# 583phoenix-hue/Airfoil-CFD-Tool

Hardware: AMD Instinct MI355X
Metric: MLUPS on 4096² fp32 D2Q9 at 1/2/4/8 MI355X; achieved % HBM3E peak (higher is better)
Workload: dtype f32

## Files before the change

airfoil-cfd-tool_amd/csrc/step_march.hpp:

```cpp
#pragma once
#include <hip/hip_runtime.h>
#include <stdint.h>
#include <algorithm>
#include <vector>
#include "step_fast.hpp"

#ifndef WT_LOAD_AUX
#define WT_LOAD_AUX 2
#endif
#ifndef WT_STORE_AUX
#define WT_STORE_AUX 2
#endif

namespace wt {

static constexpr int MARCH_MAX_CHUNK = 60;
static constexpr int MARCH3_MAX_CHUNK = 124;
static inline int march_max_len(int depth) { return depth == 4 ? MARCH3_MAX_CHUNK - 3 : (depth == 3 ? MARCH3_MAX_CHUNK : MARCH_MAX_CHUNK); }

struct ClassMask { unsigned long long lo, hi; };
__device__ __forceinline__ bool cm_bit(const ClassMask &m, int idx) { return (((idx < 64) ? (m.lo >> idx) : (m.hi >> (idx - 64))) & 1ULL) != 0; }

enum : uint8_t { WC_FAST = 0, WC_GENERAL = 1, WC_SOLID = 2 };

// ... 241 lines not shown

template <typename T, int S>
__device__ __forceinline__ void march_load_aligned(const MarchAddr<T, S> &a, int col, MV<T, S> (&fin)[9])
{
    fin[0] = bload<T, S>(a.rs, a.voff, lat_off(a, 0, col, 0));
    fin[1] = bload<T, S>(a.rs, a.voff, lat_off(a, 1, col - 1, 0));
    fin[3] = bload<T, S>(a.rs, a.voff, lat_off(a, 3, col + 1, 0));
    fin[2] = bload<T, S>(a.rs, a.voff, lat_off(a, 2, col, 0));
    fin[5] = bload<T, S>(a.rs, a.voff, lat_off(a, 5, col - 1, 0));
    fin[6] = bload<T, S>(a.rs, a.voff, lat_off(a, 6, col + 1, 0));
    fin[4] = bload<T, S>(a.rs, a.voff, lat_off(a, 4, col, 0));
    fin[7] = bload<T, S>(a.rs, a.voff, lat_off(a, 7, col + 1, 0));
    fin[8] = bload<T, S>(a.rs, a.voff, lat_off(a, 8, col - 1, 0));
}

template <int S> __device__ __forceinline__ uint32_t load_site_bytes(const uint8_t *p)
{
    if constexpr (S == 4) return *reinterpret_cast<const uint32_t *>(p);
    else if constexpr (S == 2) return *reinterpret_cast<const uint16_t *>(p);
    else return *p;
}

struct SiteBytes { uint32_t v[2]; };
template <int S, bool OVL> __device__ __forceinline__ int site_row(int j0, int ny)
{
    if constexpr (OVL) return j0 < 0 ? 0 : (j0 > ny - S ? ny - S : j0);
    else return j0;
}
template <typename T, int S, bool OVL = false>
__device__ __forceinline__ SiteBytes site_bytes_load(const MarchParams<T> &p, int col, int j0)
{
    const int c = col < 0 ? 0 : (col > p.g.nxl - 1 ? p.g.nxl - 1 : col);
    const int jb = site_row<S, OVL>(j0, p.g.ny);
    SiteBytes r;
    r.v[0] = load_site_bytes<S>(p.mask + (long)(c + 1) * p.g.pitch + jb);
    r.v[1] = load_site_bytes<S>(p.bcode + (long)c * p.g.pitch + jb);
    return r;
}

static constexpr int MARCH_FD_PACKED = 4;
typedef float f2v __attribute__((ext_vector_type(2)));
__device__ __forceinline__ f2v div2_ieee(f2v a, f2v b)
{
    bool s0, s1, dummy;
    const f2v ds = {__builtin_amdgcn_div_scalef(a[0], b[0], false, &dummy), __builtin_amdgcn_div_scalef(a[1], b[1], false, &dummy)};
    const f2v ns = {__builtin_amdgcn_div_scalef(a[0], b[0], true, &s0), __builtin_amdgcn_div_scalef(a[1], b[1], true, &s1)};
    const f2v rc = {__builtin_amdgcn_rcpf(ds[0]), __builtin_amdgcn_rcpf(ds[1])};
    const f2v one = {1.0f, 1.0f};
    const f2v f0 = __builtin_elementwise_fma(-ds, rc, one);
    const f2v f1 = __builtin_elementwise_fma(f0, rc, rc);
    const f2v mu = ns * f1;
// ... 254 lines not shown
#pragma unroll
    for (int k = 0; k < 9; k++) {
        const unsigned soff = lat_off(a, k, col, 0) - (OVL ? 256u : 0u);
        __builtin_amdgcn_raw_ptr_buffer_load_lds(a.rs, (lds_void_p)(buf + 512 * k), 4, a.voff_dma, soff, 0, 0);
        __builtin_amdgcn_raw_ptr_buffer_load_lds(a.rs, (lds_void_p)(buf + 512 * k), 4, a.voff_dma, soff, 256, 0);
    }
}
template <typename T, int S>
__device__ __forceinline__ MV<T, S> own_read(const char *buf, int k, int lane)
{
    MV<T, S> o;
    const u2v x = *reinterpret_cast<const u2v *>(buf + 512 * k + 8 * lane);
    __builtin_memcpy(&o, &x, 8);
    return o;
}

template <bool BODY, int FD, typename T, int S, bool OWN_LDS = false>
__device__ __forceinline__ void march_step1(const MarchParams<T> &p, const MarchAddr<T, S> &a, int x, int j0, bool far_win, bool nonfast, bool allsolid,
                                            const T (&feq0)[9], MV<T, S> (&in)[9], MV<T, S> (&G)[9], const uint32_t *pre = nullptr, const char *own_buf = nullptr)
{
    MV<T, S> mac[3];
    if (BODY) {
        const Geom &g = p.g;
        const int gi = x + g.gi0;
#ifdef WT_EXP_NO_OWN
        auto own = [&](int k) { return in[k]; };
#else
        auto own = [&](int k) {
            if constexpr (OWN_LDS) return own_read<T, S>(own_buf, k, a.lane);
            else return bload<T, S>(a.rs, a.voff, lat_off(a, k, x, 0));
        };
#endif
        if (__builtin_expect(gi <= 0 || gi >= g.nx_g - 1 || nonfast, 0)) {
            uint32_t solid4 = 0, code4 = 0;
            if (nonfast) {
                if (pre) { solid4 = pre[0]; code4 = pre[1]; }
                else {
                    solid4 = load_site_bytes<S>(p.mask + (long)(x + 1) * g.pitch + site_row<S, (FD & MARCH_FD_OVL) != 0>(j0, g.ny));
                    code4 = load_site_bytes<S>(p.bcode + (long)x * g.pitch + site_row<S, (FD & MARCH_FD_OVL) != 0>(j0, g.ny));
                }
            }
            const bool any_solid = __ballot(solid4 != 0) != 0ULL;
            if (gi <= 0) {
#pragma unroll
                for (int k = 0; k < 9; k++) G[k] = mv_splat<T, S>(feq0[k]);
            } else if (gi >= g.nx_g - 1) {
#pragma unroll
                for (int k = 0; k < 9; k++) G[k] = bload<T, S>(a.rs, a.voff, lat_off(a, k, x - 1, 0));
            } else if (allsolid) {
#pragma unroll
                for (int k = 0; k < 9; k++) G[k] = own(opp_of(k));
                return;
            } else {
                march_bounce<T, S>(in, code4, own);
                march_collide_general<T, S, FD, false>(in, solid4, j0, g.ny, p.fdv, p.tau, p.U0, feq0, G, mac);
                return;
            }
            if (any_solid) march_solid<T, S, false>(G, mac, solid4, own);
            return;
        }
    }
    march_collide<T, S, FD, false>(in, p.fdv, p.tau, G, mac);
    if (far_win) march_far_rows<T, S, false>(j0, p.g.ny, p.U0, feq0, G, mac);
}

struct MarchRange { int i_begin, i_end, outlet_after; };
static inline MarchRange march_range(const Geom &g)
{
    MarchRange r;
    r.i_begin = (g.gi0 == 0) ? 0 : 1;
    r.i_end = g.nxl - 1;
    r.outlet_after = (g.gi0 + g.nxl == g.nx_g) ? 1 : 0;
    return r;
// ... 128 lines not shown
```

airfoil-cfd-tool_amd/csrc/step_march3.hpp:

```cpp
#pragma once
#include "step_march.hpp"

namespace wt {

static constexpr int M3_SREC = 80;
static constexpr int M3_SHALF = 40;
static constexpr int M3_HL = 32;
static constexpr int HL_COLS = 60;
static constexpr int H3_COLS = HL_COLS, H4_COLS = HL_COLS;


__global__ __launch_bounds__(256) void k_seam_flags3(const uint8_t *__restrict__ mask, const uint8_t *__restrict__ bcode, uint8_t *__restrict__ flags3,
                                                     Geom g, int nwin, int win)
{
    const long total = (long)(nwin - 1) * g.nxl;
    const long t = (long)blockIdx.x * 256 + threadIdx.x;
    if (t >= total) return;
    const int x = (int)(t % g.nxl);
    const int b = 1 + (int)(t / g.nxl);
    const uint8_t *m = mask + g.pitch;
    const int gi = x + g.gi0;
    unsigned f = 0;
    for (int r4 = 0; r4 < 4; r4++) {
        const int j = win * b - 2 + r4;
// ... 281 lines not shown
                                            const T (&feq0)[9], const MV<T, S> (&m158)[3], const MV<T, S> (&Gc)[9], const MV<T, S> (&Gn)[9], T hv,
                                            MV<T, S> (&out)[9], MV<T, S> (&mac)[3], const uint32_t *pre = nullptr)
{
    typedef MV<T, S> V3;
    const Geom &g = p.g;
    constexpr bool OVL = (FD & MARCH_FD_OVL) != 0;
    V3 fin[9];
    fin[0] = Gc[0]; fin[1] = m158[0]; fin[3] = Gn[3];
    fin[2] = m_below_x<LB, OVL>(Gc[2], hv); fin[5] = m_below_x<LB + 1, OVL>(m158[1], hv); fin[6] = m_below_x<LB + 2, OVL>(Gn[6], hv);
    fin[4] = m_above_x<LB, OVL>(Gc[4], hv); fin[8] = m_above_x<LB + 2, OVL>(m158[2], hv); fin[7] = m_above_x<LB + 1, OVL>(Gn[7], hv);
    if (BODY) {
        const int gi = c + g.gi0;
        if (__builtin_expect(gi <= 0 || nf, 0)) {
            auto ownc = [&](int k) { return Gc[k]; };
            uint32_t solid4 = 0, code4 = 0;
            if (nf) {
                if (pre) { solid4 = pre[0]; code4 = pre[1]; }
                else {
                    solid4 = load_site_bytes<S>(p.mask + (long)(c + 1) * g.pitch + site_row<S, OVL>(j0, g.ny));
                    code4 = load_site_bytes<S>(p.bcode + (long)c * g.pitch + site_row<S, OVL>(j0, g.ny));
                }
            }
            const bool any_solid = __ballot(solid4 != 0) != 0ULL;
            if (gi <= 0) {
#pragma unroll
                for (int k = 0; k < 9; k++) out[k] = mv_splat<T, S>(feq0[k]);
                if (WANT_MACRO) { mac[0] = mv_splat<T, S>(T(1)); mac[1] = mv_splat<T, S>(p.U0); mac[2] = mv_splat<T, S>(T(0)); }
            } else if (allsolid) {
#pragma unroll
                for (int k = 0; k < 9; k++) out[k] = Gc[k];
                if (WANT_MACRO) { mac[0] = mv_splat<T, S>(T(1)); mac[1] = mv_splat<T, S>(T(0)); mac[2] = mv_splat<T, S>(T(0)); }
            } else {
                march_bounce<T, S>(fin, code4, ownc);
                march_collide_general<T, S, FD, WANT_MACRO>(fin, solid4, j0, g.ny, p.fdv, p.tau, p.U0, feq0, out, mac);
            }
            if (any_solid && (gi <= 0 || allsolid)) march_solid<T, S, WANT_MACRO>(out, mac, solid4, ownc);
            return;
// ... 87 lines not shown

template <bool BODY, bool EMIT, int FD, typename T, int S>
__device__ __forceinline__ void march_unit3(const MarchParams<T> &p, March3Addr<T, S> &m, __amdgpu_buffer_rsrc_t rh, unsigned hoff,
                                            int ia, int ib, int uflags, int j0, int lane, bool far_win, ClassMask nonfast_m,
                                            ClassMask solid_m, const T (&feq0)[9])
{
    constexpr bool OVLF = (FD & MARCH_FD_OVL) != 0;
    typedef MV<T, S> V3;
    constexpr unsigned HREC = M3_HL * sizeof(T);
    const Geom &g = p.g;
    const MarchAddr<T, S> &a = m.a;
#define NONFAST(x) (BODY && cm_bit(nonfast_m, (x) - ia + 2))
#define ALLSOLID(x) (BODY && cm_bit(solid_m, (x) - ia + 2))
#define OWN_BUF(x) (a.own_lds + ((x) & 1) * OWN_LDS_BYTES)
#define OWN_NOW(x) do { if (BODY && NONFAST(x)) own_prefetch<T, S, OVLF>(a, (x), OWN_BUF(x)); } while (0)
#define STEP1(x, in, G) march_step1<BODY, FD, T, S, BODY>(p, a, (x), j0, far_win, NONFAST(x), ALLSOLID(x), feq0, in, G, nullptr, OWN_BUF(x))
#define STEP1P(x, in, G, sb) march_step1<BODY, FD, T, S, BODY>(p, a, (x), j0, far_win, NONFAST(x), ALLSOLID(x), feq0, in, G, BODY ? (sb).v : nullptr, OWN_BUF(x))
    const bool outlet = BODY && (uflags & MU_OUTLET_AFTER) != 0;
    const int xend = outlet ? ib : ib + 1;
    V3 s1m[3], s1c[9];
    V3 s2m[3], s2c[9];
    V3 in[9], G1[9], G2[9], mac[3];
#pragma unroll
    for (int k = 0; k < 9; k++) { s1c[k] = mv_splat<T, S>(feq0[k]); s2c[k] = s1c[k]; }
    s1m[0] = s1c[1]; s1m[1] = s1c[5]; s1m[2] = s1c[8];
    s2m[0] = s1c[1]; s2m[1] = s1c[5]; s2m[2] = s1c[8];
    T hv2 = halo_load_x<OVLF, T>(rh, hoff, (unsigned)(ia - 2 > 0 ? ia - 2 : 0) * HREC);
    T hv1 = halo_load_x<OVLF, T>(rh, hoff, (unsigned)(ia - 1 > 0 ? ia - 1 : 0) * HREC);
    T hv0 = halo_load_x<OVLF, T>(rh, hoff, (unsigned)ia * HREC);
    if (!BODY || ia - 2 + g.gi0 >= 0) {
        OWN_NOW(ia - 2);
        march_load_aligned(a, ia - 2, in);
        march_align_in<OVLF>(in, lane, hv2);
        STEP1(ia - 2, in, s1c);
    }
    s1m[0] = s1c[1]; s1m[1] = s1c[5]; s1m[2] = s1c[8];
    if (!BODY || ia - 1 + g.gi0 >= 0) {
        OWN_NOW(ia - 1);
        march_load_aligned(a, ia - 1, in);
        march_align_in<OVLF>(in, lane, hv1);
        STEP1(ia - 1, in, s1c);
    }
    OWN_NOW(ia);
    march_load_aligned(a, ia, in);
    SiteBytes sb0{{0, 0}}, sb1{{0, 0}}, sb2{{0, 0}};
    if (BODY) { sb0 = site_bytes_load<T, S, OVLF>(p, ia, j0); sb1 = site_bytes_load<T, S, OVLF>(p, ia - 1, j0); sb2 = site_bytes_load<T, S, OVLF>(p, ia - 2, j0); wait_for_bytes(sb0); wait_for_bytes(sb1); wait_for_bytes(sb2); }
    wait_for_column(in, hv0, hv1, hv2);
    int seam_col = -1;
#ifdef WT_M3_STAMPS
    unsigned long long st_[8] = {0, 0, 0, 0, 0, 0, 0, 0}, tprev_ = __builtin_amdgcn_s_memtime();
#endif
#pragma unroll 1
    for (int x = ia; x <= xend; x++) {
        V3 nxt[9];
        if (BODY && x + 1 <= xend && NONFAST(x + 1)) own_prefetch<T, S, OVLF>(a, x + 1, OWN_BUF(x + 1));
        march_load_aligned(a, (x + 1 <= xend) ? x + 1 : x, nxt);
        const bool has2 = x - 2 >= ia;
        const int c1 = x - 1, c2 = x - 2;
        const T hvn = halo_load_x<OVLF, T>(rh, hoff, (unsigned)(x + 1) * HREC);
        SiteBytes sbn{{0, 0}};
        if (BODY) sbn = site_bytes_load<T, S, OVLF>(p, x + 1, j0);
        const Seam3 sp = seam3_fetch<OVLF>(m);
        M3_STAMP(0);
        march_align_in<OVLF>(in, lane, hv0);
        STEP1P(x, in, G1, sb0);
        M3_STAMP(1);
        march_stage<BODY, false, FD, 0>(p, c1, j0, lane, far_win, NONFAST(c1), ALLSOLID(c1), feq0, s1m, s1c, G1, hv1, G2, mac, BODY ? sb1.v : nullptr);
#ifdef WT_M3_STAMPS
        pin_after(G2);
#endif
        M3_STAMP(2);
        V3 out[9];
        march_stage<BODY, EMIT, FD, 4>(p, c2, j0, lane, far_win, NONFAST(c2), ALLSOLID(c2), feq0, s2m, s2c, G2, hv2, out, mac, BODY ? sb2.v : nullptr);
        pin_after(out);
        M3_STAMP(3);
        wait_for_column(nxt, hvn);
        if (BODY) { wait_for_bytes(sbn); sb2 = sb1; sb1 = sb0; sb0 = sbn; }
#ifdef WT_M3_STAMPS
        asm volatile("s_waitcnt vmcnt(0)" ::: "memory");
#endif
        M3_STAMP(4);
        hv2 = hv1; hv1 = hv0; hv0 = hvn;
        march3_store<EMIT, OVLF>(m, has2 ? a.voff_st : p.lat_bytes, has2 ? c2 : 0, out, mac);
        seam3_flush<OVLF>(m, seam_col, sp);
        M3_STAMP(5);
        seam_col = has2 ? c2 : seam_col;
        if (BODY && outlet && x == xend) break;
        s2m[0] = s2c[1]; s2m[1] = s2c[5]; s2m[2] = s2c[8];
        s1m[0] = s1c[1]; s1m[1] = s1c[5]; s1m[2] = s1c[8];
#pragma unroll
        for (int k = 0; k < 9; k++) { s2c[k] = G2[k]; s1c[k] = G1[k]; in[k] = nxt[k]; }
    }
#ifdef WT_M3_STAMPS
    if (!BODY && lane == 0) {
        for (int i = 0; i < 6; i++) atomicAdd(&g_m3_stamps[i], st_[i]);
        atomicAdd(&g_m3_stamps[6], (unsigned long long)(xend - ia + 1));
        atomicAdd(&g_m3_stamps[7], 1ULL);
    }
#endif
    if (BODY && outlet) {
        const int co = ib;
        uint32_t solid4 = 0;
        if (NONFAST(co)) solid4 = load_site_bytes<S>(p.mask + (long)(co + 1) * g.pitch + site_row<S, OVLF>(j0, g.ny));
        const bool any_solid = __ballot(solid4 != 0) != 0ULL;
        V3 L2o[9], out[9];
#pragma unroll
        for (int k = 0; k < 9; k++) L2o[k] = s1c[k];
        if (any_solid) { auto own1 = [&](int k) { return G1[k]; }; march_solid<T, S, false>(L2o, mac, solid4, own1); }
        V3 t2m[3];
        t2m[0] = s2c[1]; t2m[1] = s2c[5]; t2m[2] = s2c[8];
        const T hv2t = halo_load_x<OVLF, T>(rh, hoff, (unsigned)(co - 1) * HREC);
        Seam3 sp = seam3_fetch<OVLF>(m);
        march_stage<BODY, EMIT, FD, 4>(p, co - 1, j0, lane, far_win, NONFAST(co - 1), ALLSOLID(co - 1), feq0, t2m, G2, L2o, hv2t, out, mac);
        march3_store<EMIT, OVLF>(m, a.voff_st, co - 1, out, mac);
        seam3_flush<OVLF>(m, seam_col, sp);
        seam_col = co - 1;
#pragma unroll
        for (int k = 0; k < 9; k++) out[k] = G2[k];
        if (EMIT) march_outlet_macro(G2, mac);
        if (any_solid) { auto own2 = [&](int k) { return L2o[k]; }; march_solid<T, S, EMIT>(out, mac, solid4, own2); }
        sp = seam3_fetch<OVLF>(m);
        march3_store<EMIT, OVLF>(m, a.voff_st, co, out, mac);
        seam3_flush<OVLF>(m, seam_col, sp);
        seam_col = co;
    }
    seam3_flush<OVLF>(m, seam_col, seam3_fetch<OVLF>(m));
#undef NONFAST
#undef ALLSOLID
#undef STEP1
#undef STEP1P
#undef OWN_BUF
#undef OWN_NOW
}

template <bool BODY, bool EMIT, int FD, typename T, int S>
__device__ __forceinline__ void march_unit4(const MarchParams<T> &p, March3Addr<T, S> &m, __amdgpu_buffer_rsrc_t rh,
                                            unsigned hoff, int ia, int ib, int uflags, int j0, int lane, bool far_win,
                                            ClassMask nonfast_m, ClassMask solid_m, const T (&feq0)[9])
{
    constexpr bool OVLF = (FD & MARCH_FD_OVL) != 0;
    typedef MV<T, S> V3;
    constexpr unsigned HREC = M3_HL * sizeof(T);
    const Geom &g = p.g;
    const MarchAddr<T, S> &a = m.a;
#define NONFAST(x) (BODY && (x) >= ia - 3 && cm_bit(nonfast_m, (x) - ia + 3))
#define ALLSOLID(x) (BODY && (x) >= ia - 3 && cm_bit(solid_m, (x) - ia + 3))
#define OWN_BUF(x) (a.own_lds + ((x) & 1) * OWN_LDS_BYTES)
#define OWN_NOW(x) do { if (BODY && NONFAST(x)) own_prefetch<T, S, OVLF>(a, (x), OWN_BUF(x)); } while (0)
#define STEP1(x, in, G) march_step1<BODY, FD, T, S, BODY>(p, a, (x), j0, far_win, NONFAST(x), ALLSOLID(x), feq0, in, G, nullptr, OWN_BUF(x))
#define HCOL(c) ((unsigned)((c) > 0 ? (c) : 0) * HREC)
    const bool outlet = BODY && (uflags & MU_OUTLET_AFTER) != 0;
    const int xend = outlet ? ib : ib + 2;
    V3 s1m[3], s1c[9];
    V3 s2m[3], s2c[9];
    V3 s3m[3], s3c[9];
    V3 in[9], G1[9], G2[9], G3[9], mac[3];
#pragma unroll
    for (int k = 0; k < 9; k++) { s1c[k] = mv_splat<T, S>(feq0[k]); s2c[k] = s1c[k]; s3c[k] = s1c[k]; }
    s1m[0] = s1c[1]; s1m[1] = s1c[5]; s1m[2] = s1c[8];
    s2m[0] = s1c[1]; s2m[1] = s1c[5]; s2m[2] = s1c[8];
    s3m[0] = s1c[1]; s3m[1] = s1c[5]; s3m[2] = s1c[8];
    const int xs = ia - 1;
#define LCOL(x) ((BODY && (x) + g.gi0 < 0) ? -g.gi0 : (x))
    T hv3 = halo_load_x<OVLF, T>(rh, hoff, HCOL(xs - 3)), hv2 = halo_load_x<OVLF, T>(rh, hoff, HCOL(xs - 2)), hv1 = halo_load_x<OVLF, T>(rh, hoff, HCOL(xs - 1)),
// ... 3 lines not shown
        march_load_aligned(a, ia - 3, in);
        march_align_in<OVLF>(in, lane, hv2);
        STEP1(ia - 3, in, s1c);
    }
    s1m[0] = s1c[1]; s1m[1] = s1c[5]; s1m[2] = s1c[8];
    if (!BODY || ia - 2 + g.gi0 >= 0) {
        OWN_NOW(ia - 2);
        march_load_aligned(a, ia - 2, in);
        march_align_in<OVLF>(in, lane, hv1);
        STEP1(ia - 2, in, s1c);
    }
    OWN_NOW(xs);
    march_load_aligned(a, LCOL(xs), in);
    SiteBytes sb0{{0, 0}}, sb1{{0, 0}}, sb2{{0, 0}}, sb3{{0, 0}};
    if (BODY) {
        sb0 = site_bytes_load<T, S, OVLF>(p, xs, j0); sb1 = site_bytes_load<T, S, OVLF>(p, xs - 1, j0); sb2 = site_bytes_load<T, S, OVLF>(p, xs - 2, j0); sb3 = site_bytes_load<T, S, OVLF>(p, xs - 3, j0);
        wait_for_bytes(sb0); wait_for_bytes(sb1); wait_for_bytes(sb2); wait_for_bytes(sb3);
    }
    wait_for_column(in, hv0, hv1, hv2);
    wait_for_column(in, hv3);
    int seam_col = -1;
#pragma unroll 1
    for (int x = xs; x <= xend; x++) {
        V3 nxt[9];
        if (BODY && x + 1 <= xend && NONFAST(x + 1)) own_prefetch<T, S, OVLF>(a, x + 1, OWN_BUF(x + 1));
        march_load_aligned(a, (x + 1 <= xend) ? x + 1 : x, nxt);
        const bool has3 = x - 3 >= ia;
        const int c1 = x - 1, c2 = x - 2, c3 = x - 3;
        const T hvn = halo_load_x<OVLF, T>(rh, hoff, HCOL(x + 1));
        SiteBytes sbn{{0, 0}};
        if (BODY) sbn = site_bytes_load<T, S, OVLF>(p, x + 1, j0);
        const Seam3 sp = seam3_fetch<OVLF>(m);
        march_align_in<OVLF>(in, lane, hv0);
        march_step1<BODY, FD, T, S, BODY>(p, a, x, j0, far_win, NONFAST(x), ALLSOLID(x), feq0, in, G1, BODY ? sb0.v : nullptr, OWN_BUF(x));

        march_stage<BODY, false, FD, 0>(p, c1, j0, lane, far_win, NONFAST(c1), ALLSOLID(c1), feq0, s1m, s1c, G1, hv1, G2, mac, BODY ? sb1.v : nullptr);
        march_stage<BODY, false, FD, 4>(p, c2, j0, lane, far_win, NONFAST(c2), ALLSOLID(c2), feq0, s2m, s2c, G2, hv2, G3, mac, BODY ? sb2.v : nullptr);
        V3 out[9];
        march_stage<BODY, EMIT, FD, 8>(p, c3, j0, lane, far_win, NONFAST(c3), ALLSOLID(c3), feq0, s3m, s3c, G3, hv3, out, mac, BODY ? sb3.v : nullptr);
        pin_after(out);
        wait_for_column(nxt, hvn);
        if (BODY) { wait_for_bytes(sbn); sb3 = sb2; sb2 = sb1; sb1 = sb0; sb0 = sbn; }
        hv3 = hv2; hv2 = hv1; hv1 = hv0; hv0 = hvn;
        march3_store<EMIT, OVLF>(m, has3 ? a.voff_st : p.lat_bytes, has3 ? c3 : 0, out, mac);
        seam3_flush<OVLF>(m, seam_col, sp);
        seam_col = has3 ? c3 : seam_col;
        if (BODY && outlet && x == xend) break;
        s3m[0] = s3c[1]; s3m[1] = s3c[5]; s3m[2] = s3c[8];
        s2m[0] = s2c[1]; s2m[1] = s2c[5]; s2m[2] = s2c[8];
        s1m[0] = s1c[1]; s1m[1] = s1c[5]; s1m[2] = s1c[8];
#pragma unroll
        for (int k = 0; k < 9; k++) { s3c[k] = G3[k]; s2c[k] = G2[k]; s1c[k] = G1[k]; in[k] = nxt[k]; }
    }
    if (BODY && outlet) {
        const int co = ib;
        uint32_t solid4 = 0;
        if (NONFAST(co)) solid4 = load_site_bytes<S>(p.mask + (long)(co + 1) * g.pitch + site_row<S, OVLF>(j0, g.ny));
        const bool any_solid = __ballot(solid4 != 0) != 0ULL;
        V3 O2[9], O3[9], L3a[9], out[9], tm[3];
#pragma unroll
        for (int k = 0; k < 9; k++) O2[k] = s1c[k];
        if (any_solid) { auto own = [&](int k) { return G1[k]; }; march_solid<T, S, false>(O2, mac, solid4, own); }
        tm[0] = s2c[1]; tm[1] = s2c[5]; tm[2] = s2c[8];
        march_stage<BODY, false, FD, 4>(p, co - 1, j0, lane, far_win, NONFAST(co - 1), ALLSOLID(co - 1), feq0, tm, G2, O2, halo_load_x<OVLF, T>(rh, hoff, HCOL(co - 1)), L3a, mac);
#pragma unroll
        for (int k = 0; k < 9; k++) O3[k] = G2[k];
        if (any_solid) { auto own = [&](int k) { return O2[k]; }; march_solid<T, S, false>(O3, mac, solid4, own); }
        tm[0] = s3c[1]; tm[1] = s3c[5]; tm[2] = s3c[8];
        Seam3 sp = seam3_fetch<OVLF>(m);
        const bool own2 = co - 2 >= ia;
        march_stage<BODY, EMIT, FD, 8>(p, co - 2, j0, lane, far_win, NONFAST(co - 2), ALLSOLID(co - 2), feq0, tm, G3, L3a, halo_load_x<OVLF, T>(rh, hoff, HCOL(co - 2)), out, mac);
        march3_store<EMIT, OVLF>(m, own2 ? a.voff_st : p.lat_bytes, own2 ? co - 2 : 0, out, mac);
        seam3_flush<OVLF>(m, seam_col, sp);
        seam_col = own2 ? co - 2 : seam_col;
        tm[0] = G3[1]; tm[1] = G3[5]; tm[2] = G3[8];
        sp = seam3_fetch<OVLF>(m);
        march_stage<BODY, EMIT, FD, 8>(p, co - 1, j0, lane, far_win, NONFAST(co - 1), ALLSOLID(co - 1), feq0, tm, L3a, O3, halo_load_x<OVLF, T>(rh, hoff, HCOL(co - 1)), out, mac);
        march3_store<EMIT, OVLF>(m, a.voff_st, co - 1, out, mac);
        seam3_flush<OVLF>(m, seam_col, sp);
        seam_col = co - 1;
#pragma unroll
        for (int k = 0; k < 9; k++) out[k] = L3a[k];
        if (EMIT) march_outlet_macro(L3a, mac);
        if (any_solid) { auto own = [&](int k) { return O3[k]; }; march_solid<T, S, EMIT>(out, mac, solid4, own); }
        sp = seam3_fetch<OVLF>(m);
        march3_store<EMIT, OVLF>(m, a.voff_st, co, out, mac);
        seam3_flush<OVLF>(m, seam_col, sp);
        seam_col = co;
    }
    seam3_flush<OVLF>(m, seam_col, seam3_fetch<OVLF>(m));
#undef NONFAST
#undef ALLSOLID
#undef STEP1
#undef OWN_BUF
#undef OWN_NOW
#undef HCOL
#undef LCOL
}

template <bool BODY, bool EMIT, int FD, typename T, int S>
__device__ __forceinline__ void march_unit3_d2(const MarchParams<T> &p, March3Addr<T, S> &m, __amdgpu_buffer_rsrc_t rh, unsigned hoff, int ia, int ib,
                                               int uflags, int j0, int lane, bool far_win, ClassMask nonfast_m, ClassMask solid_m,
                                               const T (&feq0)[9])
{
    constexpr bool OVLF = (FD & MARCH_FD_OVL) != 0;
    typedef MV<T, S> V3;
    constexpr unsigned HREC = M3_HL * sizeof(T);
    const Geom &g = p.g;
    const MarchAddr<T, S> &a = m.a;
#define NONFAST(x) (BODY && cm_bit(nonfast_m, (x) - ia + 2))
#define ALLSOLID(x) (BODY && cm_bit(solid_m, (x) - ia + 2))
#define STEP1(x, in, G) march_step1<BODY, FD, T, S>(p, a, (x), j0, far_win, NONFAST(x), ALLSOLID(x), feq0, in, G)
    const bool outlet = BODY && (uflags & MU_OUTLET_AFTER) != 0;
    const int xend = ib;
    V3 s1m[3], s1c[9];
    V3 in[9], G1[9], mac[3];
#pragma unroll
    for (int k = 0; k < 9; k++) s1c[k] = mv_splat<T, S>(feq0[k]);
    s1m[0] = s1c[1]; s1m[1] = s1c[5]; s1m[2] = s1c[8];
    T hv1 = halo_load_x<OVLF, T>(rh, hoff, (unsigned)(ia - 1 > 0 ? ia - 1 : 0) * HREC), hv0 = halo_load_x<OVLF, T>(rh, hoff, (unsigned)ia * HREC);
    if (!BODY || ia - 1 + g.gi0 >= 0) {
        march_load_aligned(a, ia - 1, in);
        march_align_in<OVLF>(in, lane, hv1);
        STEP1(ia - 1, in, s1c);
    }
    march_load_aligned(a, ia, in);
    wait_for_column(in, hv0, hv1);
    int seam_col = -1;
#pragma unroll 1
    for (int x = ia; x <= xend; x++) {
        V3 nxt[9];
        march_load_aligned(a, (x + 1 <= xend) ? x + 1 : x, nxt);
        const bool has1 = x - 1 >= ia;
        const int c1 = x - 1;
        const T hvn = halo_load_x<OVLF, T>(rh, hoff, (unsigned)(x + 1) * HREC);
        const Seam3 sp = seam3_fetch<OVLF>(m);
        march_align_in<OVLF>(in, lane, hv0);
        STEP1(x, in, G1);
        V3 out[9];
        march_stage<BODY, EMIT, FD, 0>(p, c1, j0, lane, far_win, NONFAST(c1), ALLSOLID(c1), feq0, s1m, s1c, G1, hv1, out, mac);
        pin_after(out);
        wait_for_column(nxt, hvn);
        hv1 = hv0; hv0 = hvn;
        march3_store<EMIT, OVLF>(m, has1 ? a.voff_st : p.lat_bytes, has1 ? c1 : 0, out, mac);
        seam3_flush<OVLF>(m, seam_col, sp);
        seam_col = has1 ? c1 : seam_col;
        if (BODY && outlet && x == xend) break;
        s1m[0] = s1c[1]; s1m[1] = s1c[5]; s1m[2] = s1c[8];
#pragma unroll
        for (int k = 0; k < 9; k++) { s1c[k] = G1[k]; in[k] = nxt[k]; }
    }
    if (BODY && outlet) {
        const int co = ib;
        uint32_t solid4 = 0;
        if (NONFAST(co)) solid4 = load_site_bytes<S>(p.mask + (long)(co + 1) * g.pitch + site_row<S, OVLF>(j0, g.ny));
        V3 out[9];
#pragma unroll
        for (int k = 0; k < 9; k++) out[k] = s1c[k];
        if (EMIT) march_outlet_macro(s1c, mac);
        if (__ballot(solid4 != 0) != 0ULL) { auto own1 = [&](int k) { return G1[k]; }; march_solid<T, S, EMIT>(out, mac, solid4, own1); }
        const Seam3 sp = seam3_fetch<OVLF>(m);
        march3_store<EMIT, OVLF>(m, a.voff_st, co, out, mac);
        seam3_flush<OVLF>(m, seam_col, sp);
        seam_col = co;
    }
    seam3_flush<OVLF>(m, seam_col, seam3_fetch<OVLF>(m));
#undef NONFAST
#undef ALLSOLID
#undef STEP1
}

static inline MarchRange march_range3(const Geom &g, int depth = 3)
{
    MarchRange r;
    r.i_begin = (g.gi0 == 0) ? 0 : depth - 1;
    r.outlet_after = (g.gi0 + g.nxl == g.nx_g) ? 1 : 0;
    r.i_end = r.outlet_after ? g.nxl - 1 : g.nxl - (depth - 1);
    return r;
}

}
```

Measured before the change: 219,900.

## Route site-byte loads through buffer resources and prefetch own-populations via LDS everywhere

Mask and boundary-code bytes are now read with raw buffer loads from a per-window resource descriptor rather than flat global pointers. The depth-2 march also gets LDS prefetch of own populations and pipelined site bytes, matching the other depths. Non-fast and all-solid flags are carried in rolling bitmasks instead of being re-derived from class masks, and outlet paths reuse already-loaded site bytes. A counted-waitcnt inline-asm path pairs LDS reads for bounce-back, which trades more register pressure and asm fragility for fewer per-column wait stalls.

Result: slower. 217,200 (-1.2%).

```diff
diff --git a/airfoil-cfd-tool_amd/csrc/step_march.hpp b/airfoil-cfd-tool_amd/csrc/step_march.hpp
--- a/airfoil-cfd-tool_amd/csrc/step_march.hpp
+++ b/airfoil-cfd-tool_amd/csrc/step_march.hpp
@@ -2,6 +2,7 @@
 #include <hip/hip_runtime.h>
 #include <stdint.h>
 #include <algorithm>
+#include <type_traits>
 #include <vector>
 #include "step_fast.hpp"
 
@@ -279,27 +280,38 @@
     fin[8] = bload<T, S>(a.rs, a.voff, lat_off(a, 8, col - 1, 0));
 }
 
-template <int S> __device__ __forceinline__ uint32_t load_site_bytes(const uint8_t *p)
-{
-    if constexpr (S == 4) return *reinterpret_cast<const uint32_t *>(p);
-    else if constexpr (S == 2) return *reinterpret_cast<const uint16_t *>(p);
-    else return *p;
-}
-
 struct SiteBytes { uint32_t v[2]; };
 template <int S, bool OVL> __device__ __forceinline__ int site_row(int j0, int ny)
 {
     if constexpr (OVL) return j0 < 0 ? 0 : (j0 > ny - S ? ny - S : j0);
     else return j0;
 }
+struct SiteSrc { __amdgpu_buffer_rsrc_t rmask, rcode; unsigned voff, pitch; int last; };
 template <typename T, int S, bool OVL = false>
-__device__ __forceinline__ SiteBytes site_bytes_load(const MarchParams<T> &p, int col, int j0)
-{
-    const int c = col < 0 ? 0 : (col > p.g.nxl - 1 ? p.g.nxl - 1 : col);
-    const int jb = site_row<S, OVL>(j0, p.g.ny);
+__device__ __forceinline__ SiteSrc site_src(const MarchParams<T> &p, int j0)
+{
+    SiteSrc s;
+    const unsigned bytes = (unsigned)(p.g.nxl + 2) * (unsigned)p.g.pitch;
+    s.rmask = march_rsrc(p.mask, bytes);
+    s.rcode = march_rsrc(p.bcode, bytes);
+    s.voff = (unsigned)site_row<S, OVL>(j0, p.g.ny);
+    s.pitch = (unsigned)p.g.pitch;
+    s.last = p.g.nxl - 1;
+    return s;
+}
+template <int S> __device__ __forceinline__ uint32_t load_site_bytes(__amdgpu_buffer_rsrc_t r, unsigned voff, unsigned soff)
+{
+    if constexpr (S == 4) return __builtin_amdgcn_raw_buffer_load_b32(r, voff, soff, 0);
+    else if constexpr (S == 2) return __builtin_amdgcn_raw_buffer_load_b16(r, voff, soff, 0);
+    else return __builtin_amdgcn_raw_buffer_load_b8(r, voff, soff, 0);
+}
+template <int S>
+__device__ __forceinline__ SiteBytes site_bytes_load(const SiteSrc &s, int col)
+{
+    const int c = col < 0 ? 0 : (col > s.last ? s.last : col);
     SiteBytes r;
-    r.v[0] = load_site_bytes<S>(p.mask + (long)(c + 1) * p.g.pitch + jb);
-    r.v[1] = load_site_bytes<S>(p.bcode + (long)c * p.g.pitch + jb);
+    r.v[0] = load_site_bytes<S>(s.rmask, s.voff, (unsigned)(c + 1) * s.pitch);
+    r.v[1] = load_site_bytes<S>(s.rcode, s.voff, (unsigned)c * s.pitch);
     return r;
 }
 
@@ -584,8 +596,66 @@
     __builtin_memcpy(&o, &x, 8);
     return o;
 }
-
-template <bool BODY, int FD, typename T, int S, bool OWN_LDS = false>
+static constexpr int OWN_VMCNT = 32;
+typedef __attribute__((address_space(3))) char *lds_char_p;
+__device__ __forceinline__ unsigned own_lds_addr(const char *buf, int lane) { return (unsigned)(size_t)(lds_char_p)buf + 8u * (unsigned)lane; }
+template <int A, int B, bool FIRST, typename T, int S>
+__device__ __forceinline__ void own_pair_counted(unsigned addr, MV<T, S> &oa, MV<T, S> &ob)
+{
+    static_assert(S * sizeof(T) == 8, "one 8-byte read per lane and population");
+    u4v pr;
+    if constexpr (FIRST)
+        asm volatile("s_waitcnt vmcnt(%4)\n\tds_read2st64_b64 %0, %1 offset0:%2 offset1:%3\n\ts_waitcnt lgkmcnt(0)" : "=&v"(pr) : "v"(addr), "n"(A), "n"(B), "n"(OWN_VMCNT));
+    else
+        asm volatile("ds_read2st64_b64 %0, %1 offset0:%2 offset1:%3\n\ts_waitcnt lgkmcnt(0)" : "=&v"(pr) : "v"(addr), "n"(A), "n"(B));
+    const u2v qa = {pr.x, pr.y}, qb = {pr.z, pr.w};
+    __builtin_memcpy(&oa, &qa, 8);
+    __builtin_memcpy(&ob, &qb, 8);
+}
+template <typename T, int S>
+__device__ __forceinline__ void march_bounce_counted(MV<T, S> (&fin)[9], uint32_t code4, unsigned addr)
+{
+    auto pair = [&](auto first, auto ca, auto cb) {
+        constexpr int A = decltype(ca)::value, B = decltype(cb)::value;
+        MV<T, S> oa, ob;
+        own_pair_counted<A, B, decltype(first)::value>(addr, oa, ob);
+#pragma unroll
+        for (int v = 0; v < S; v++) {
+            fin[A].v[v] = ((code4 >> (8 * v + A - 1)) & 1u) ? ob.v[v] : fin[A].v[v];
+            fin[B].v[v] = ((code4 >> (8 * v + B - 1)) & 1u) ? oa.v[v] : fin[B].v[v];
+        }
+    };
+    typedef std::integral_constant<bool, true> Y;
+    typedef std::integral_constant<bool, false> N;
+    pair(Y{}, std::integral_constant<int, 1>{}, std::integral_constant<int, 3>{});
+    pair(N{}, std::integral_constant<int, 2>{}, std::integral_constant<int, 4>{});
+    pair(N{}, std::integral_constant<int, 5>{}, std::integral_constant<int, 7>{});
+    pair(N{}, std::integral_constant<int, 6>{}, std::integral_constant<int, 8>{});
+}
+template <bool ALL, typename T, int S>
+__device__ __forceinline__ void march_reverse_counted(MV<T, S> (&G)[9], uint32_t solid4, unsigned addr)
+{
+    auto put = [&](MV<T, S> &g, const MV<T, S> &o) {
+#pragma unroll
+        for (int v = 0; v < S; v++) g.v[v] = (ALL || ((solid4 >> (8 * v)) & 0xffu)) ? o.v[v] : g.v[v];
+    };
+    auto pair = [&](auto first, auto ca, auto cb) {
+        constexpr int A = decltype(ca)::value, B = decltype(cb)::value;
+        MV<T, S> oa, ob;
+        own_pair_counted<A, B, decltype(first)::value>(addr, oa, ob);
+        if constexpr (A == 0) put(G[0], oa);
+        else { put(G[A], ob); put(G[B], oa); }
+    };
+    typedef std::integral_constant<bool, true> Y;
+    typedef std::integral_constant<bool, false> N;
+    pair(Y{}, std::integral_constant<int, 1>{}, std::integral_constant<int, 3>{});
+    pair(N{}, std::integral_constant<int, 2>{}, std::integral_constant<int, 4>{});
+    pair(N{}, std::integral_constant<int, 5>{}, std::integral_constant<int, 7>{});
+    pair(N{}, std::integral_constant<int, 6>{}, std::integral_constant<int, 8>{});
+    pair(N{}, std::integral_constant<int, 0>{}, std::integral_constant<int, 1>{});
+}
+
+template <bool BODY, int FD, typename T, int S, bool OWN_COUNTED = false>
 __device__ __forceinline__ void march_step1(const MarchParams<T> &p, const MarchAddr<T, S> &a, int x, int j0, bool far_win, bool nonfast, bool allsolid,
                                             const T (&feq0)[9], MV<T, S> (&in)[9], MV<T, S> (&G)[9], const uint32_t *pre = nullptr, const char *own_buf = nullptr)
 {
@@ -593,23 +663,10 @@
     if (BODY) {
         const Geom &g = p.g;
         const int gi = x + g.gi0;
-#ifdef WT_EXP_NO_OWN
-        auto own = [&](int k) { return in[k]; };
-#else
-        auto own = [&](int k) {
-            if constexpr (OWN_LDS) return own_read<T, S>(own_buf, k, a.lane);
-            else return bload<T, S>(a.rs, a.voff, lat_off(a, k, x, 0));
-        };
-#endif
+        auto own = [&](int k) { return own_read<T, S>(own_buf, k, a.lane); };
         if (__builtin_expect(gi <= 0 || gi >= g.nx_g - 1 || nonfast, 0)) {
             uint32_t solid4 = 0, code4 = 0;
-            if (nonfast) {
-                if (pre) { solid4 = pre[0]; code4 = pre[1]; }
-                else {
-                    solid4 = load_site_bytes<S>(p.mask + (long)(x + 1) * g.pitch + site_row<S, (FD & MARCH_FD_OVL) != 0>(j0, g.ny));
-                    code4 = load_site_bytes<S>(p.bcode + (long)x * g.pitch + site_row<S, (FD & MARCH_FD_OVL) != 0>(j0, g.ny));
-                }
-            }
+            if (nonfast) { solid4 = pre[0]; code4 = pre[1]; }
             const bool any_solid = __ballot(solid4 != 0) != 0ULL;
             if (gi <= 0) {
 #pragma unroll
@@ -617,16 +674,29 @@
             } else if (gi >= g.nx_g - 1) {
 #pragma unroll
                 for (int k = 0; k < 9; k++) G[k] = bload<T, S>(a.rs, a.voff, lat_off(a, k, x - 1, 0));
+                if constexpr ((FD & MARCH_FD_CONTRACTED) == 0) {
+                    u2v r[9];
+#pragma unroll
+                    for (int k = 0; k < 9; k++) __builtin_memcpy(&r[k], &G[k], 8);
+                    asm volatile("" ::"v"(r[0]), "v"(r[1]), "v"(r[2]), "v"(r[3]), "v"(r[4]), "v"(r[5]), "v"(r[6]), "v"(r[7]), "v"(r[8]));
+                }
             } else if (allsolid) {
-#pragma unroll
-                for (int k = 0; k < 9; k++) G[k] = own(opp_of(k));
+                if constexpr (OWN_COUNTED) march_reverse_counted<true, T, S>(G, 0u, own_lds_addr(own_buf, a.lane));
+                else {
+#pragma unroll
+                    for (int k = 0; k < 9; k++) G[k] = own(opp_of(k));
+                }
                 return;
             } else {
-                march_bounce<T, S>(in, code4, own);
+                if constexpr (OWN_COUNTED) march_bounce_counted<T, S>(in, code4, own_lds_addr(own_buf, a.lane));
+                else march_bounce<T, S>(in, code4, own);
                 march_collide_general<T, S, FD, false>(in, solid4, j0, g.ny, p.fdv, p.tau, p.U0, feq0, G, mac);
                 return;
             }
-            if (any_solid) march_solid<T, S, false>(G, mac, solid4, own);
+            if (any_solid) {
+                if constexpr (OWN_COUNTED) march_reverse_counted<false, T, S>(G, solid4, own_lds_addr(own_buf, a.lane));
+                else march_solid<T, S, false>(G, mac, solid4, own);
+            }
             return;
         }
     }
diff --git a/airfoil-cfd-tool_amd/csrc/step_march3.hpp b/airfoil-cfd-tool_amd/csrc/step_march3.hpp
--- a/airfoil-cfd-tool_amd/csrc/step_march3.hpp
+++ b/airfoil-cfd-tool_amd/csrc/step_march3.hpp
@@ -319,13 +319,7 @@
         if (__builtin_expect(gi <= 0 || nf, 0)) {
             auto ownc = [&](int k) { return Gc[k]; };
             uint32_t solid4 = 0, code4 = 0;
-            if (nf) {
-                if (pre) { solid4 = pre[0]; code4 = pre[1]; }
-                else {
-                    solid4 = load_site_bytes<S>(p.mask + (long)(c + 1) * g.pitch + site_row<S, OVL>(j0, g.ny));
-                    code4 = load_site_bytes<S>(p.bcode + (long)c * g.pitch + site_row<S, OVL>(j0, g.ny));
-                }
-            }
+            if (nf) { solid4 = pre[0]; code4 = pre[1]; }
             const bool any_solid = __ballot(solid4 != 0) != 0ULL;
             if (gi <= 0) {
 #pragma unroll
@@ -443,8 +437,11 @@
 #define ALLSOLID(x) (BODY && cm_bit(solid_m, (x) - ia + 2))
 #define OWN_BUF(x) (a.own_lds + ((x) & 1) * OWN_LDS_BYTES)
 #define OWN_NOW(x) do { if (BODY && NONFAST(x)) own_prefetch<T, S, OVLF>(a, (x), OWN_BUF(x)); } while (0)
-#define STEP1(x, in, G) march_step1<BODY, FD, T, S, BODY>(p, a, (x), j0, far_win, NONFAST(x), ALLSOLID(x), feq0, in, G, nullptr, OWN_BUF(x))
-#define STEP1P(x, in, G, sb) march_step1<BODY, FD, T, S, BODY>(p, a, (x), j0, far_win, NONFAST(x), ALLSOLID(x), feq0, in, G, BODY ? (sb).v : nullptr, OWN_BUF(x))
+#define STEP1(x, in, G) do { SiteBytes sb_{{0, 0}}; if (BODY) sb_ = site_bytes_load<S>(ss, (x)); \
+                             march_step1<BODY, FD, T, S>(p, a, (x), j0, far_win, NONFAST(x), ALLSOLID(x), feq0, in, G, sb_.v, OWN_BUF(x)); } while (0)
+#define NFW(k) (BODY && ((nfw >> (k)) & 1u) != 0)
+#define ASW(k) (BODY && ((asw >> (k)) & 1u) != 0)
+    const SiteSrc ss = site_src<T, S, OVLF>(p, j0);
     const bool outlet = BODY && (uflags & MU_OUTLET_AFTER) != 0;
     const int xend = outlet ? ib : ib + 1;
     V3 s1m[3], s1c[9];
@@ -473,8 +470,13 @@
     OWN_NOW(ia);
     march_load_aligned(a, ia, in);
     SiteBytes sb0{{0, 0}}, sb1{{0, 0}}, sb2{{0, 0}};
-    if (BODY) { sb0 = site_bytes_load<T, S, OVLF>(p, ia, j0); sb1 = site_bytes_load<T, S, OVLF>(p, ia - 1, j0); sb2 = site_bytes_load<T, S, OVLF>(p, ia - 2, j0); wait_for_bytes(sb0); wait_for_bytes(sb1); wait_for_bytes(sb2); }
+    if (BODY) { sb0 = site_bytes_load<S>(ss, ia); sb1 = site_bytes_load<S>(ss, ia - 1); sb2 = site_bytes_load<S>(ss, ia - 2); wait_for_bytes(sb0); wait_for_bytes(sb1); wait_for_bytes(sb2); }
     wait_for_column(in, hv0, hv1, hv2);
+    unsigned nfw = 0, asw = 0;
+    if (BODY) {
+        nfw = (NONFAST(ia) ? 1u : 0u) | (NONFAST(ia - 1) ? 2u : 0u) | (NONFAST(ia - 2) ? 4u : 0u);
+        asw = (ALLSOLID(ia) ? 1u : 0u) | (ALLSOLID(ia - 1) ? 2u : 0u) | (ALLSOLID(ia - 2) ? 4u : 0u);
+    }
     int seam_col = -1;
 #ifdef WT_M3_STAMPS
     unsigned long long st_[8] = {0, 0, 0, 0, 0, 0, 0, 0}, tprev_ = __builtin_amdgcn_s_memtime();
@@ -482,29 +484,30 @@
 #pragma unroll 1
     for (int x = ia; x <= xend; x++) {
         V3 nxt[9];
-        if (BODY && x + 1 <= xend && NONFAST(x + 1)) own_prefetch<T, S, OVLF>(a, x + 1, OWN_BUF(x + 1));
+        const bool nfn = BODY && x + 1 <= xend && NONFAST(x + 1), asn = BODY && x + 1 <= xend && ALLSOLID(x + 1);
+        if (nfn) own_prefetch<T, S, OVLF>(a, x + 1, OWN_BUF(x + 1));
         march_load_aligned(a, (x + 1 <= xend) ? x + 1 : x, nxt);
         const bool has2 = x - 2 >= ia;
         const int c1 = x - 1, c2 = x - 2;
         const T hvn = halo_load_x<OVLF, T>(rh, hoff, (unsigned)(x + 1) * HREC);
         SiteBytes sbn{{0, 0}};
-        if (BODY) sbn = site_bytes_load<T, S, OVLF>(p, x + 1, j0);
+        if (BODY) sbn = site_bytes_load<S>(ss, x + 1);
         const Seam3 sp = seam3_fetch<OVLF>(m);
         M3_STAMP(0);
         march_align_in<OVLF>(in, lane, hv0);
-        STEP1P(x, in, G1, sb0);
+        march_step1<BODY, FD, T, S, BODY>(p, a, x, j0, far_win, NFW(0), ASW(0), feq0, in, G1, sb0.v, OWN_BUF(x));
         M3_STAMP(1);
-        march_stage<BODY, false, FD, 0>(p, c1, j0, lane, far_win, NONFAST(c1), ALLSOLID(c1), feq0, s1m, s1c, G1, hv1, G2, mac, BODY ? sb1.v : nullptr);
+        march_stage<BODY, false, FD, 0>(p, c1, j0, lane, far_win, NFW(1), ASW(1), feq0, s1m, s1c, G1, hv1, G2, mac, sb1.v);
 #ifdef WT_M3_STAMPS
         pin_after(G2);
 #endif
         M3_STAMP(2);
         V3 out[9];
-        march_stage<BODY, EMIT, FD, 4>(p, c2, j0, lane, far_win, NONFAST(c2), ALLSOLID(c2), feq0, s2m, s2c, G2, hv2, out, mac, BODY ? sb2.v : nullptr);
+        march_stage<BODY, EMIT, FD, 4>(p, c2, j0, lane, far_win, NFW(2), ASW(2), feq0, s2m, s2c, G2, hv2, out, mac, sb2.v);
         pin_after(out);
         M3_STAMP(3);
         wait_for_column(nxt, hvn);
-        if (BODY) { wait_for_bytes(sbn); sb2 = sb1; sb1 = sb0; sb0 = sbn; }
+        if (BODY) { wait_for_bytes(sbn); sb2 = sb1; sb1 = sb0; sb0 = sbn; nfw = (nfw << 1) | (nfn ? 1u : 0u); asw = (asw << 1) | (asn ? 1u : 0u); }
 #ifdef WT_M3_STAMPS
         asm volatile("s_waitcnt vmcnt(0)" ::: "memory");
 #endif
@@ -529,8 +532,7 @@
 #endif
     if (BODY && outlet) {
         const int co = ib;
-        uint32_t solid4 = 0;
-        if (NONFAST(co)) solid4 = load_site_bytes<S>(p.mask + (long)(co + 1) * g.pitch + site_row<S, OVLF>(j0, g.ny));
+        const uint32_t solid4 = NONFAST(co) ? sb1.v[0] : 0u;
         const bool any_solid = __ballot(solid4 != 0) != 0ULL;
         V3 L2o[9], out[9];
 #pragma unroll
@@ -540,7 +542,7 @@
         t2m[0] = s2c[1]; t2m[1] = s2c[5]; t2m[2] = s2c[8];
         const T hv2t = halo_load_x<OVLF, T>(rh, hoff, (unsigned)(co - 1) * HREC);
         Seam3 sp = seam3_fetch<OVLF>(m);
-        march_stage<BODY, EMIT, FD, 4>(p, co - 1, j0, lane, far_win, NONFAST(co - 1), ALLSOLID(co - 1), feq0, t2m, G2, L2o, hv2t, out, mac);
+        march_stage<BODY, EMIT, FD, 4>(p, co - 1, j0, lane, far_win, NONFAST(co - 1), ALLSOLID(co - 1), feq0, t2m, G2, L2o, hv2t, out, mac, sb2.v);
         march3_store<EMIT, OVLF>(m, a.voff_st, co - 1, out, mac);
         seam3_flush<OVLF>(m, seam_col, sp);
         seam_col = co - 1;
@@ -557,7 +559,8 @@
 #undef NONFAST
 #undef ALLSOLID
 #undef STEP1
-#undef STEP1P
+#undef NFW
+#undef ASW
 #undef OWN_BUF
 #undef OWN_NOW
 }
@@ -576,7 +579,11 @@
 #define ALLSOLID(x) (BODY && (x) >= ia - 3 && cm_bit(solid_m, (x) - ia + 3))
 #define OWN_BUF(x) (a.own_lds + ((x) & 1) * OWN_LDS_BYTES)
 #define OWN_NOW(x) do { if (BODY && NONFAST(x)) own_prefetch<T, S, OVLF>(a, (x), OWN_BUF(x)); } while (0)
-#define STEP1(x, in, G) march_step1<BODY, FD, T, S, BODY>(p, a, (x), j0, far_win, NONFAST(x), ALLSOLID(x), feq0, in, G, nullptr, OWN_BUF(x))
+#define STEP1(x, in, G) do { SiteBytes sb_{{0, 0}}; if (BODY) sb_ = site_bytes_load<S>(ss, (x)); \
+                             march_step1<BODY, FD, T, S>(p, a, (x), j0, far_win, NONFAST(x), ALLSOLID(x), feq0, in, G, sb_.v, OWN_BUF(x)); } while (0)
+#define NFW(k) (BODY && ((nfw >> (k)) & 1u) != 0)
+#define ASW(k) (BODY && ((asw >> (k)) & 1u) != 0)
+    const SiteSrc ss = site_src<T, S, OVLF>(p, j0);
 #define HCOL(c) ((unsigned)((c) > 0 ? (c) : 0) * HREC)
     const bool outlet = BODY && (uflags & MU_OUTLET_AFTER) != 0;
     const int xend = outlet ? ib : ib + 2;
@@ -610,33 +617,39 @@
     march_load_aligned(a, LCOL(xs), in);
     SiteBytes sb0{{0, 0}}, sb1{{0, 0}}, sb2{{0, 0}}, sb3{{0, 0}};
     if (BODY) {
-        sb0 = site_bytes_load<T, S, OVLF>(p, xs, j0); sb1 = site_bytes_load<T, S, OVLF>(p, xs - 1, j0); sb2 = site_bytes_load<T, S, OVLF>(p, xs - 2, j0); sb3 = site_bytes_load<T, S, OVLF>(p, xs - 3, j0);
+        sb0 = site_bytes_load<S>(ss, xs); sb1 = site_bytes_load<S>(ss, xs - 1); sb2 = site_bytes_load<S>(ss, xs - 2); sb3 = site_bytes_load<S>(ss, xs - 3);
         wait_for_bytes(sb0); wait_for_bytes(sb1); wait_for_bytes(sb2); wait_for_bytes(sb3);
     }
     wait_for_column(in, hv0, hv1, hv2);
     wait_for_column(in, hv3);
+    unsigned nfw = 0, asw = 0;
+    if (BODY) {
+        nfw = (NONFAST(xs) ? 1u : 0u) | (NONFAST(xs - 1) ? 2u : 0u) | (NONFAST(xs - 2) ? 4u : 0u);
+        asw = (ALLSOLID(xs) ? 1u : 0u) | (ALLSOLID(xs - 1) ? 2u : 0u) | (ALLSOLID(xs - 2) ? 4u : 0u);
+    }
     int seam_col = -1;
 #pragma unroll 1
     for (int x = xs; x <= xend; x++) {
         V3 nxt[9];
-        if (BODY && x + 1 <= xend && NONFAST(x + 1)) own_prefetch<T, S, OVLF>(a, x + 1, OWN_BUF(x + 1));
+        const bool nfn = BODY && x + 1 <= xend && NONFAST(x + 1), asn = BODY && x + 1 <= xend && ALLSOLID(x + 1);
+        if (nfn) own_prefetch<T, S, OVLF>(a, x + 1, OWN_BUF(x + 1));
         march_load_aligned(a, (x + 1 <= xend) ? x + 1 : x, nxt);
         const bool has3 = x - 3 >= ia;
         const int c1 = x - 1, c2 = x - 2, c3 = x - 3;
         const T hvn = halo_load_x<OVLF, T>(rh, hoff, HCOL(x + 1));
         SiteBytes sbn{{0, 0}};
-        if (BODY) sbn = site_bytes_load<T, S, OVLF>(p, x + 1, j0);
+        if (BODY) sbn = site_bytes_load<S>(ss, x + 1);
         const Seam3 sp = seam3_fetch<OVLF>(m);
         march_align_in<OVLF>(in, lane, hv0);
-        march_step1<BODY, FD, T, S, BODY>(p, a, x, j0, far_win, NONFAST(x), ALLSOLID(x), feq0, in, G1, BODY ? sb0.v : nullptr, OWN_BUF(x));
-
-        march_stage<BODY, false, FD, 0>(p, c1, j0, lane, far_win, NONFAST(c1), ALLSOLID(c1), feq0, s1m, s1c, G1, hv1, G2, mac, BODY ? sb1.v : nullptr);
-        march_stage<BODY, false, FD, 4>(p, c2, j0, lane, far_win, NONFAST(c2), ALLSOLID(c2), feq0, s2m, s2c, G2, hv2, G3, mac, BODY ? sb2.v : nullptr);
+        march_step1<BODY, FD, T, S, BODY>(p, a, x, j0, far_win, NFW(0), ASW(0), feq0, in, G1, sb0.v, OWN_BUF(x));
+
+        march_stage<BODY, false, FD, 0>(p, c1, j0, lane, far_win, NFW(1), ASW(1), feq0, s1m, s1c, G1, hv1, G2, mac, sb1.v);
+        march_stage<BODY, false, FD, 4>(p, c2, j0, lane, far_win, NFW(2), ASW(2), feq0, s2m, s2c, G2, hv2, G3, mac, sb2.v);
         V3 out[9];
-        march_stage<BODY, EMIT, FD, 8>(p, c3, j0, lane, far_win, NONFAST(c3), ALLSOLID(c3), feq0, s3m, s3c, G3, hv3, out, mac, BODY ? sb3.v : nullptr);
+        march_stage<BODY, EMIT, FD, 8>(p, c3, j0, lane, far_win, NFW(3), ASW(3), feq0, s3m, s3c, G3, hv3, out, mac, sb3.v);
         pin_after(out);
         wait_for_column(nxt, hvn);
-        if (BODY) { wait_for_bytes(sbn); sb3 = sb2; sb2 = sb1; sb1 = sb0; sb0 = sbn; }
+        if (BODY) { wait_for_bytes(sbn); sb3 = sb2; sb2 = sb1; sb1 = sb0; sb0 = sbn; nfw = (nfw << 1) | (nfn ? 1u : 0u); asw = (asw << 1) | (asn ? 1u : 0u); }
         hv3 = hv2; hv2 = hv1; hv1 = hv0; hv0 = hvn;
         march3_store<EMIT, OVLF>(m, has3 ? a.voff_st : p.lat_bytes, has3 ? c3 : 0, out, mac);
         seam3_flush<OVLF>(m, seam_col, sp);
@@ -650,28 +663,27 @@
     }
     if (BODY && outlet) {
         const int co = ib;
-        uint32_t solid4 = 0;
-        if (NONFAST(co)) solid4 = load_site_bytes<S>(p.mask + (long)(co + 1) * g.pitch + site_row<S, OVLF>(j0, g.ny));
+        const uint32_t solid4 = NONFAST(co) ? sb1.v[0] : 0u;
         const bool any_solid = __ballot(solid4 != 0) != 0ULL;
         V3 O2[9], O3[9], L3a[9], out[9], tm[3];
 #pragma unroll
         for (int k = 0; k < 9; k++) O2[k] = s1c[k];
         if (any_solid) { auto own = [&](int k) { return G1[k]; }; march_solid<T, S, false>(O2, mac, solid4, own); }
         tm[0] = s2c[1]; tm[1] = s2c[5]; tm[2] = s2c[8];
-        march_stage<BODY, false, FD, 4>(p, co - 1, j0, lane, far_win, NONFAST(co - 1), ALLSOLID(co - 1), feq0, tm, G2, O2, halo_load_x<OVLF, T>(rh, hoff, HCOL(co - 1)), L3a, mac);
+        march_stage<BODY, false, FD, 4>(p, co - 1, j0, lane, far_win, NONFAST(co - 1), ALLSOLID(co - 1), feq0, tm, G2, O2, halo_load_x<OVLF, T>(rh, hoff, HCOL(co - 1)), L3a, mac, sb2.v);
 #pragma unroll
         for (int k = 0; k < 9; k++) O3[k] = G2[k];
         if (any_solid) { auto own = [&](int k) { return O2[k]; }; march_solid<T, S, false>(O3, mac, solid4, own); }
         tm[0] = s3c[1]; tm[1] = s3c[5]; tm[2] = s3c[8];
         Seam3 sp = seam3_fetch<OVLF>(m);
         const bool own2 = co - 2 >= ia;
-        march_stage<BODY, EMIT, FD, 8>(p, co - 2, j0, lane, far_win, NONFAST(co - 2), ALLSOLID(co - 2), feq0, tm, G3, L3a, halo_load_x<OVLF, T>(rh, hoff, HCOL(co - 2)), out, mac);
+        march_stage<BODY, EMIT, FD, 8>(p, co - 2, j0, lane, far_win, NONFAST(co - 2), ALLSOLID(co - 2), feq0, tm, G3, L3a, halo_load_x<OVLF, T>(rh, hoff, HCOL(co - 2)), out, mac, sb3.v);
         march3_store<EMIT, OVLF>(m, own2 ? a.voff_st : p.lat_bytes, own2 ? co - 2 : 0, out, mac);
         seam3_flush<OVLF>(m, seam_col, sp);
         seam_col = own2 ? co - 2 : seam_col;
         tm[0] = G3[1]; tm[1] = G3[5]; tm[2] = G3[8];
         sp = seam3_fetch<OVLF>(m);
-        march_stage<BODY, EMIT, FD, 8>(p, co - 1, j0, lane, far_win, NONFAST(co - 1), ALLSOLID(co - 1), feq0, tm, L3a, O3, halo_load_x<OVLF, T>(rh, hoff, HCOL(co - 1)), out, mac);
+        march_stage<BODY, EMIT, FD, 8>(p, co - 1, j0, lane, far_win, NONFAST(co - 1), ALLSOLID(co - 1), feq0, tm, L3a, O3, halo_load_x<OVLF, T>(rh, hoff, HCOL(co - 1)), out, mac, sb2.v);
         march3_store<EMIT, OVLF>(m, a.voff_st, co - 1, out, mac);
         seam3_flush<OVLF>(m, seam_col, sp);
         seam_col = co - 1;
@@ -688,6 +700,8 @@
 #undef NONFAST
 #undef ALLSOLID
 #undef STEP1
+#undef NFW
+#undef ASW
 #undef OWN_BUF
 #undef OWN_NOW
 #undef HCOL
@@ -706,7 +720,13 @@
     const MarchAddr<T, S> &a = m.a;
 #define NONFAST(x) (BODY && cm_bit(nonfast_m, (x) - ia + 2))
 #define ALLSOLID(x) (BODY && cm_bit(solid_m, (x) - ia + 2))
-#define STEP1(x, in, G) march_step1<BODY, FD, T, S>(p, a, (x), j0, far_win, NONFAST(x), ALLSOLID(x), feq0, in, G)
+#define OWN_BUF(x) (a.own_lds + ((x) & 1) * OWN_LDS_BYTES)
+#define OWN_NOW(x) do { if (BODY && NONFAST(x)) own_prefetch<T, S, OVLF>(a, (x), OWN_BUF(x)); } while (0)
+#define STEP1(x, in, G) do { SiteBytes sb_{{0, 0}}; if (BODY) sb_ = site_bytes_load<S>(ss, (x)); \
+                             march_step1<BODY, FD, T, S>(p, a, (x), j0, far_win, NONFAST(x), ALLSOLID(x), feq0, in, G, sb_.v, OWN_BUF(x)); } while (0)
+#define NFW(k) (BODY && ((nfw >> (k)) & 1u) != 0)
+#define ASW(k) (BODY && ((asw >> (k)) & 1u) != 0)
+    const SiteSrc ss = site_src<T, S, OVLF>(p, j0);
     const bool outlet = BODY && (uflags & MU_OUTLET_AFTER) != 0;
     const int xend = ib;
     V3 s1m[3], s1c[9];
@@ -716,27 +736,41 @@
     s1m[0] = s1c[1]; s1m[1] = s1c[5]; s1m[2] = s1c[8];
     T hv1 = halo_load_x<OVLF, T>(rh, hoff, (unsigned)(ia - 1 > 0 ? ia - 1 : 0) * HREC), hv0 = halo_load_x<OVLF, T>(rh, hoff, (unsigned)ia * HREC);
     if (!BODY || ia - 1 + g.gi0 >= 0) {
+        OWN_NOW(ia - 1);
         march_load_aligned(a, ia - 1, in);
         march_align_in<OVLF>(in, lane, hv1);
         STEP1(ia - 1, in, s1c);
     }
+    OWN_NOW(ia);
     march_load_aligned(a, ia, in);
+    SiteBytes sb0{{0, 0}}, sb1{{0, 0}};
+    if (BODY) { sb0 = site_bytes_load<S>(ss, ia); sb1 = site_bytes_load<S>(ss, ia - 1); wait_for_bytes(sb0); wait_for_bytes(sb1); }
     wait_for_column(in, hv0, hv1);
+    unsigned nfw = 0, asw = 0;
+    if (BODY) {
+        nfw = (NONFAST(ia) ? 1u : 0u) | (NONFAST(ia - 1) ? 2u : 0u);
+        asw = (ALLSOLID(ia) ? 1u : 0u) | (ALLSOLID(ia - 1) ? 2u : 0u);
+    }
     int seam_col = -1;
 #pragma unroll 1
     for (int x = ia; x <= xend; x++) {
         V3 nxt[9];
+        const bool nfn = BODY && x + 1 <= xend && NONFAST(x + 1), asn = BODY && x + 1 <= xend && ALLSOLID(x + 1);
+        if (nfn) own_prefetch<T, S, OVLF>(a, x + 1, OWN_BUF(x + 1));
         march_load_aligned(a, (x + 1 <= xend) ? x + 1 : x, nxt);
         const bool has1 = x - 1 >= ia;
         const int c1 = x - 1;
         const T hvn = halo_load_x<OVLF, T>(rh, hoff, (unsigned)(x + 1) * HREC);
+        SiteBytes sbn{{0, 0}};
+        if (BODY) sbn = site_bytes_load<S>(ss, x + 1);
         const Seam3 sp = seam3_fetch<OVLF>(m);
         march_align_in<OVLF>(in, lane, hv0);
-        STEP1(x, in, G1);
+        march_step1<BODY, FD, T, S, BODY>(p, a, x, j0, far_win, NFW(0), ASW(0), feq0, in, G1, sb0.v, OWN_BUF(x));
         V3 out[9];
-        march_stage<BODY, EMIT, FD, 0>(p, c1, j0, lane, far_win, NONFAST(c1), ALLSOLID(c1), feq0, s1m, s1c, G1, hv1, out, mac);
+        march_stage<BODY, EMIT, FD, 0>(p, c1, j0, lane, far_win, NFW(1), ASW(1), feq0, s1m, s1c, G1, hv1, out, mac, sb1.v);
         pin_after(out);
         wait_for_column(nxt, hvn);
+        if (BODY) { wait_for_bytes(sbn); sb1 = sb0; sb0 = sbn; nfw = (nfw << 1) | (nfn ? 1u : 0u); asw = (asw << 1) | (asn ? 1u : 0u); }
         hv1 = hv0; hv0 = hvn;
         march3_store<EMIT, OVLF>(m, has1 ? a.voff_st : p.lat_bytes, has1 ? c1 : 0, out, mac);
         seam3_flush<OVLF>(m, seam_col, sp);
@@ -748,8 +782,7 @@
     }
     if (BODY && outlet) {
         const int co = ib;
-        uint32_t solid4 = 0;
-        if (NONFAST(co)) solid4 = load_site_bytes<S>(p.mask + (long)(co + 1) * g.pitch + site_row<S, OVLF>(j0, g.ny));
+        const uint32_t solid4 = NONFAST(co) ? sb1.v[0] : 0u;
         V3 out[9];
 #pragma unroll
         for (int k = 0; k < 9; k++) out[k] = s1c[k];
@@ -764,6 +797,10 @@
 #undef NONFAST
 #undef ALLSOLID
 #undef STEP1
+#undef NFW
+#undef ASW
+#undef OWN_BUF
+#undef OWN_NOW
 }
 
 static inline MarchRange march_range3(const Geom &g, int depth = 3)
```
